# amiezzi/narrow_band_least_squares

Measured on AMD Instinct MI355X. Metric: (window x band) LTS solves/sec, 8-element synthetic, higher is better.
Workload: dtype f64

## Files before the change

include/nbls.h:

```cpp
#ifndef NBLS_H
#define NBLS_H

#include <stdint.h>

#ifdef __cplusplus
extern "C" {
#endif

typedef struct nbls_handle nbls_handle;

typedef enum {
    NBLS_OK = 0,
    NBLS_ERR_ARG = -1,
    NBLS_ERR_STATE = -2,
    NBLS_ERR_GEOMETRY = -3,
    NBLS_ERR_HIP = -4,
    NBLS_ERR_NOMEM = -5,
    NBLS_ERR_UNSUPPORTED = -6,
    NBLS_ERR_COMM = -7
} nbls_status;

typedef struct {
    double alpha;
    int32_t h;
// ... 82 lines not shown
int nbls_comm_unique_id(void* id, int32_t nbytes);
int nbls_comm_init_rank(nbls_handle* h, const void* id, int32_t world, int32_t rank);
int nbls_reserve_results(nbls_handle* h, int64_t bytes);
int nbls_comm_gather(nbls_handle* const* hs, int32_t n, int32_t root, int64_t block_bytes, int64_t status,
                     void* host_out, int64_t host_bytes);
int nbls_load_result_block(nbls_handle* h, const void* block, int64_t nbytes);
int nbls_comm_destroy(nbls_handle* h);

int nbls_set_option(nbls_handle* h, const char* key, int64_t value);
int nbls_developer_build(void);

enum {
    NBLS_ROUTE_REJECTED = 0,
    NBLS_ROUTE_SCREEN = 1,
    NBLS_ROUTE_MFMA = 2,
    NBLS_ROUTE_VALU_LDS = 3,
    NBLS_ROUTE_VALU_GLOBAL = 4
};
enum { NBLS_ROUTE_QUANTIZE = 0, NBLS_ROUTE_SCREEN_STAGE = 1, NBLS_ROUTE_VERIFY = 2, NBLS_ROUTE_GENERAL = 3 };
enum { NBLS_ROUTE_OPT_NC4 = 1, NBLS_ROUTE_OPT_NSL1 = 2, NBLS_ROUTE_OPT_TB8 = 4, NBLS_ROUTE_OPT_TB4 = 8 };
typedef struct {
    int32_t correlator;
    int32_t impl;
    int32_t ncopy, G, S, nsl;
    int32_t PFB, CSB, CSA, WP;
    int32_t screen_inst;
    int32_t tab_lds;
    int32_t quant_inst;
    int32_t quant_waves;
    int32_t verifier;
    int32_t verify_threads;
    int64_t lds_dyn[4];
    int64_t lds_static[4];
} nbls_route;
int nbls_route_xcorr(int32_t nelem, int32_t W, int32_t npairs, int32_t vrows, int64_t npts_pad, int32_t xcorr_impl,
                     int32_t flags, nbls_route* out);
int nbls_route_table(int32_t nelem, int32_t W0, int32_t W1, int32_t npairs, int32_t vrows, int64_t npts_pad,
                     int32_t xcorr_impl, int32_t flags, nbls_route* out);

int nbls_set_profiling(nbls_handle* h, int32_t on);
int nbls_get_timings(nbls_handle* h, nbls_timings* out);

int nbls_run(nbls_handle* h, int32_t nbands, const double* sos, int32_t nsections,
             int32_t zero_phase, const double* taper_left, const double* taper_right,
             int32_t taper_len, const int32_t* winlen, const int32_t* wininc,
             int32_t vector_len, const nbls_lts_params* lts, int32_t xcorr_impl,
             double* vel, double* baz, double* mdccm, double* sigma_tau, int32_t* nwin,
             int32_t* lag, double* cmax, uint8_t* weights, double* z);

int nbls_probe_mfma_f64(nbls_handle* h, const double* a, const double* b, double* out);
int nbls_probe_mfma_i8(nbls_handle* h, const int32_t* a, const int32_t* b, int32_t* out);

int nbls_debug_screen_stats(nbls_handle* h, int64_t* out8);
int nbls_debug_lts_stamps(nbls_handle* h, double* out8);
int nbls_debug_lts_coop_breakdown(nbls_handle* h, double* out8);
int nbls_debug_screen_stamps(nbls_handle* h, double* out10);

#ifdef __cplusplus
}
#endif
#endif
```

narrow_band_least_squares_amd/_hip.py:

```python
import ctypes as C
import os

import numpy as np

_HERE = os.path.dirname(os.path.abspath(__file__))
LIB_PATH = os.environ.get('NBLS_LIB') or os.path.join(_HERE, 'csrc', 'libnbls_hip.so')

EXPORTS = [
    'nbls_version', 'nbls_device_count', 'nbls_create', 'nbls_destroy', 'nbls_last_error', 'nbls_set_trace',
    'nbls_set_geometry', 'nbls_plan', 'nbls_execute', 'nbls_execute_stages', 'nbls_execute_after', 'nbls_set_trace_shape', 'nbls_upload_rows', 'nbls_sync',
    'nbls_fetch', 'nbls_fetch_filtered', 'nbls_device_results', 'nbls_set_profiling',
    'nbls_get_timings', 'nbls_run', 'nbls_probe_mfma_f64', 'nbls_probe_mfma_i8', 'nbls_debug_screen_stats', 'nbls_set_window_ranges', 'nbls_debug_screen_stamps', 'nbls_debug_lts_stamps',
    'nbls_set_trace_rows', 'nbls_result_layout', 'nbls_fetch_packed', 'nbls_comm_init_all', 'nbls_comm_unique_id',
    'nbls_comm_init_rank', 'nbls_reserve_results', 'nbls_comm_gather', 'nbls_comm_destroy', 'nbls_set_option',
    'nbls_developer_build', 'nbls_set_trace_from', 'nbls_debug_lts_coop_breakdown', 'nbls_filter_segment',
    'nbls_set_filtered', 'nbls_load_result_block', 'nbls_stream_results', 'nbls_result_batches', 'nbls_wait_result_batch',
    'nbls_comm_set_library', 'nbls_set_uncertainty', 'nbls_fetch_uncertainty', 'nbls_expect_upload', 'nbls_abort_upload',
    'nbls_set_segments', 'nbls_route_xcorr', 'nbls_route_table',
]

NBLS_ERR_ARG, NBLS_ERR_STATE, NBLS_ERR_GEOMETRY = -1, -2, -3
NBLS_ERR_HIP, NBLS_ERR_NOMEM, NBLS_ERR_UNSUPPORTED, NBLS_ERR_COMM = -4, -5, -6, -7


class NblsError(RuntimeError):
    def __init__(self, code, msg):
        super().__init__('libnbls_hip error %d: %s' % (code, msg))
        self.code = code


class LtsParams(C.Structure):
    _fields_ = [
        ('alpha', C.c_double), ('h', C.c_int32), ('nstarts', C.c_int32),
        ('starts', C.POINTER(C.c_int32)), ('csteps', C.c_int32), ('csteps2', C.c_int32),
        ('ncand', C.c_int32), ('xij_mad', C.c_double * 2), ('raw_factor', C.c_double),
        ('rew_table', C.POINTER(C.c_double)), ('quantile', C.c_double), ('zero_scale', C.c_double),
    ]


class Timings(C.Structure):
    _fields_ = [('filter_ms', C.c_double), ('xcorr_ms', C.c_double), ('solve_ms', C.c_double),
                ('total_ms', C.c_double), ('xcorr_launches', C.c_int64), ('quantize_ms', C.c_double),
                ('screen_ms', C.c_double), ('verify_ms', C.c_double), ('xcorr_impl', C.c_int32),
                ('xcorr_fallback_bands', C.c_int32)]


ROUTE_REJECTED, ROUTE_SCREEN, ROUTE_MFMA, ROUTE_VALU_LDS, ROUTE_VALU_GLOBAL = 0, 1, 2, 3, 4
ROUTE_QUANTIZE, ROUTE_SCREEN_STAGE, ROUTE_VERIFY, ROUTE_GENERAL = 0, 1, 2, 3
ROUTE_OPT_NC4, ROUTE_OPT_NSL1, ROUTE_OPT_TB8, ROUTE_OPT_TB4 = 1, 2, 4, 8
ROUTE_DTYPE = np.dtype([(k, np.int32) for k in ('correlator', 'impl', 'ncopy', 'G', 'S', 'nsl', 'PFB', 'CSB', 'CSA', 'WP',
                                                 'screen_inst', 'tab_lds', 'quant_inst', 'quant_waves', 'verifier',
                                                 'verify_threads')] +
                       [('lds_dyn', np.int64, (4,)), ('lds_static', np.int64, (4,))])
ROUTE_KEYS = ('correlator', 'ncopy', 'G', 'S', 'nsl', 'screen_inst', 'tab_lds', 'quant_inst', 'quant_waves', 'verifier',
              'verify_threads')


class Route(C.Structure):
    _fields_ = [(k, C.c_int32) for k in ROUTE_DTYPE.names[:16]] + [('lds_dyn', C.c_int64 * 4), ('lds_static', C.c_int64 * 4)]


_lib = None


def load_library(path=None):
    global _lib
    if _lib is not None and path is None:
        return _lib
    p = path or LIB_PATH
    if not os.path.exists(p):
        raise ImportError('%s not found: build it with `make -C %s` (or __graft_entry__.build()); '
# ... 2 lines not shown
    dp = C.POINTER(C.c_double)
    ip = C.POINTER(C.c_int32)
    u8p = C.POINTER(C.c_uint8)
    vp = C.c_void_p
    lib.nbls_version.restype = C.c_int
    lib.nbls_create.argtypes = [C.c_int, C.POINTER(vp)]
    lib.nbls_destroy.argtypes = [vp]
    lib.nbls_destroy.restype = None
    lib.nbls_last_error.argtypes = [vp]
    lib.nbls_last_error.restype = C.c_char_p
    lib.nbls_set_trace.argtypes = [vp, dp, C.c_int32, C.c_int64, C.c_double]
    lib.nbls_set_trace_rows.argtypes = [vp, C.POINTER(C.c_void_p), C.c_int32, C.c_int64, C.c_double]
    lib.nbls_result_layout.argtypes = [vp, C.POINTER(C.c_int64)]
    lib.nbls_fetch_packed.argtypes = [vp, C.c_void_p, C.c_int64]
    lib.nbls_comm_init_all.argtypes = [C.POINTER(vp), C.c_int32]
    lib.nbls_comm_unique_id.argtypes = [C.c_void_p, C.c_int32]
    lib.nbls_comm_init_rank.argtypes = [vp, C.c_void_p, C.c_int32, C.c_int32]
    lib.nbls_reserve_results.argtypes = [vp, C.c_int64]
    lib.nbls_load_result_block.argtypes = [vp, C.c_void_p, C.c_int64]
    lib.nbls_comm_gather.argtypes = [C.POINTER(vp), C.c_int32, C.c_int32, C.c_int64, C.c_int64, C.c_void_p, C.c_int64]
    lib.nbls_comm_destroy.argtypes = [vp]
    lib.nbls_expect_upload.argtypes = [vp]
    lib.nbls_abort_upload.argtypes = [vp]
    lib.nbls_comm_set_library.argtypes = [C.c_char_p, C.c_int32]
    lib.nbls_set_uncertainty.argtypes = [vp, dp]
    lib.nbls_fetch_uncertainty.argtypes = [vp, dp, dp]
    lib.nbls_stream_results.argtypes = [vp, C.c_int32]
    lib.nbls_result_batches.argtypes = [vp, C.POINTER(C.c_int32)]
    lib.nbls_wait_result_batch.argtypes = [vp, C.c_int32, C.POINTER(C.c_int64), C.POINTER(C.c_void_p)]
    lib.nbls_set_trace_from.argtypes = [vp, vp]
    lib.nbls_filter_segment.argtypes = [vp, C.c_int32, dp, dp]
    lib.nbls_set_filtered.argtypes = [vp, C.c_int32, dp]
    lib.nbls_set_option.argtypes = [vp, C.c_char_p, C.c_int64]
    lib.nbls_set_geometry.argtypes = [vp, dp, ip, dp, C.c_int32]
    plan_args = [vp, C.c_int32, dp, C.c_int32, C.c_int32, dp, dp, C.c_int32, ip, ip, C.c_int32,
                 C.POINTER(LtsParams), C.c_int32]
    lib.nbls_plan.argtypes = plan_args
    lib.nbls_execute.argtypes = [vp]
    lib.nbls_execute_stages.argtypes = [vp, C.c_int32]
    lib.nbls_execute_after.argtypes = [vp, vp]
    lib.nbls_set_trace_shape.argtypes = [vp, C.c_int32, C.c_int64, C.c_double]
    lib.nbls_upload_rows.argtypes = [vp, C.POINTER(C.c_void_p), C.c_int32, C.c_int64]
    lib.nbls_sync.argtypes = [vp]
    fetch_args = [dp, dp, dp, dp, ip, ip, dp, u8p, dp]
    lib.nbls_fetch.argtypes = [vp] + fetch_args
    lib.nbls_fetch_filtered.argtypes = [vp, C.c_int32, dp]
    lib.nbls_device_results.argtypes = [vp, C.POINTER(vp), C.POINTER(C.c_int64)]
    lib.nbls_set_profiling.argtypes = [vp, C.c_int32]
    lib.nbls_get_timings.argtypes = [vp, C.POINTER(Timings)]
    lib.nbls_run.argtypes = plan_args + fetch_args
    lib.nbls_probe_mfma_f64.argtypes = [vp, dp, dp, dp]
    lib.nbls_probe_mfma_i8.argtypes = [vp, ip, ip, ip]
    lib.nbls_debug_screen_stats.argtypes = [vp, C.POINTER(C.c_int64)]
    lib.nbls_set_window_ranges.argtypes = [vp, C.c_int32, ip, ip]
    lib.nbls_set_segments.argtypes = [vp, C.c_int32]
    lib.nbls_debug_screen_stamps.argtypes = [vp, dp]
    lib.nbls_debug_lts_stamps.argtypes = [vp, dp]
    lib.nbls_debug_lts_coop_breakdown.argtypes = [vp, dp]
    lib.nbls_route_xcorr.argtypes = [C.c_int32, C.c_int32, C.c_int32, C.c_int32, C.c_int64, C.c_int32, C.c_int32,
                                     C.POINTER(Route)]
    lib.nbls_route_table.argtypes = [C.c_int32, C.c_int32, C.c_int32, C.c_int32, C.c_int32, C.c_int64, C.c_int32, C.c_int32,
                                     C.c_void_p]
    for name in EXPORTS:
        if name not in ('nbls_destroy', 'nbls_last_error'):
            getattr(lib, name).restype = C.c_int
    if path is None:
        _lib = lib
    return lib


def _dptr(a):
    return None if a is None else a.ctypes.data_as(C.POINTER(C.c_double))


def _iptr(a):
    return None if a is None else a.ctypes.data_as(C.POINTER(C.c_int32))


def _u8ptr(a):
    return None if a is None else a.ctypes.data_as(C.POINTER(C.c_uint8))


def _f64(a):
    return np.ascontiguousarray(a, dtype=np.float64)


class Handle:

    def __init__(self, device_id=0):
        self.lib = load_library()
        h = C.c_void_p()
        rc = self.lib.nbls_create(int(device_id), C.byref(h))
        if rc != 0:
            raise NblsError(rc, self.lib.nbls_last_error(None).decode())
        self._h = h
        self.device_id = int(device_id)
        self.nchans = self.npts = self.npairs = 0
        self.nbands = self.vector_len = 0
        self.nseg = 1
        self._keep = []
        self.profiling = False
        self.resident_key = None

    def close(self):
        if getattr(self, '_h', None):
            self.lib.nbls_destroy(self._h)
# ... 314 lines not shown
```

narrow_band_least_squares_amd/csrc/api.hip:

```cpp
#include "nbls_internal.h"
#include <algorithm>

#include <cmath>
#include <cstdio>
#include <cstdlib>
#include <cstring>
#include <chrono>
#include <condition_variable>
#include <functional>
#include <mutex>
#include <thread>
#include <unistd.h>

namespace {

std::mutex g_err_mu;
std::string g_err;

int fail(nbls_handle* h, int code, const std::string& msg) {
    if (h) { std::lock_guard<std::mutex> l(h->err_mu); h->err = msg; }
    else { std::lock_guard<std::mutex> l(g_err_mu); g_err = msg; }
    return code;
}

// ... 294 lines not shown
    for (int i = 0; i < 4; ++i) if (h->ev[i]) (void)hipEventDestroy(h->ev[i]);
    for (hipEvent_t e : h->bev) (void)hipEventDestroy(e);
    for (hipEvent_t e : h->pev) (void)hipEventDestroy(e);
    for (hipEvent_t e : h->rev) (void)hipEventDestroy(e);
    if (h->cstream) { (void)hipStreamSynchronize(h->cstream); (void)hipStreamDestroy(h->cstream); }
    if (h->ustream) { (void)hipStreamSynchronize(h->ustream); (void)hipStreamDestroy(h->ustream); }
    for (hipEvent_t e : h->uev) (void)hipEventDestroy(e);
    if (h->ev_uprev) (void)hipEventDestroy(h->ev_uprev);
    if (h->h_res) (void)hipHostFree(h->h_res);
    if (h->ev_xd) (void)hipEventDestroy(h->ev_xd);
    if (h->ev_plan) (void)hipEventDestroy(h->ev_plan);
    if (h->ev_up) (void)hipEventDestroy(h->ev_up);
    if (h->up && h->up != h->stream) (void)hipStreamDestroy(h->up);
    if (h->stream2) (void)hipStreamDestroy(h->stream2);
    if (h->stream) (void)hipStreamDestroy(h->stream);
    if (h->stage) (void)hipHostFree(h->stage);
    delete h;
}

static void set_elements(nbls_handle* h, int32_t nchans) {
    const int E = h->nseg > 1 && nchans % h->nseg == 0 ? nchans / h->nseg : nchans;
    if (h->nelem != E && h->d_xij) {
        (void)hipFree(h->d_xij); h->d_xij = nullptr;
        h->caps.erase((const void*)&h->d_xij);
        h->npairs = 0;
    }
    h->nelem = E;
}

static int trace_shape_impl(nbls_handle* h, int32_t nchans, int64_t npts, double fs) {
    HIPCHK(h, hipSetDevice(h->device));
    const int64_t pad = (npts + 63) / 64 * 64;
    const size_t need = (size_t)nchans * pad * sizeof(double);
    if (!h->d_trace || h->cap_trace < need) {
        if (h->d_trace) { (void)hipFree(h->d_trace); h->d_trace = nullptr; h->cap_trace = 0; }
        HIPCHK(h, hipMalloc((void**)&h->d_trace, need));
        h->cap_trace = need;
    }
    set_elements(h, nchans);
    h->nchans = nchans;
    h->npts = npts;
    h->npts_pad = pad;
    h->fs = fs;
    h->planned = false;
    h->trace_loaded = false;
    h->rows_landed.store(0, std::memory_order_release);
    h->upload_state.store(2, std::memory_order_release);
    return NBLS_OK;
}

static int trace_copy_impl(nbls_handle* h, const double* const* rows, const double* flat) {
    struct Guard {
        nbls_handle* h; bool ok = false;
        ~Guard() { h->upload_state.store(ok ? 0 : -1, std::memory_order_release); }
    } guard{h};
    h->rows_landed.store(0, std::memory_order_release);
    h->upload_state.store(1, std::memory_order_release);
    HIPCHK(h, hipSetDevice(h->device));
    const int32_t nchans = h->nchans;
    const int64_t npts = h->npts, pad = h->npts_pad;
    if (!h->ustream) HIPCHK(h, hipStreamCreateWithFlags(&h->ustream, hipStreamNonBlocking));
    if (!h->ev_uprev) HIPCHK(h, hipEventCreateWithFlags(&h->ev_uprev, hipEventDisableTiming));
    while ((int)h->uev.size() < nchans) {
        hipEvent_t e;
        HIPCHK(h, hipEventCreateWithFlags(&e, hipEventDisableTiming));
        h->uev.push_back(e);
    }
    for (hipStream_t s : {h->stream, h->stream2}) {
        if (!s) continue;
        HIPCHK(h, hipEventRecord(h->ev_uprev, s));
        HIPCHK(h, hipStreamWaitEvent(h->ustream, h->ev_uprev, 0));
    }
    if (pad > npts)
        HIPCHK(h, hipMemset2DAsync(h->d_trace + npts, pad * sizeof(double), 0, (pad - npts) * sizeof(double), nchans, h->ustream));
    if (flat) {
        HIPCHK(h, hipMemcpy2DAsync(h->d_trace, pad * sizeof(double), flat, npts * sizeof(double),
                                   npts * sizeof(double), nchans, hipMemcpyHostToDevice, h->ustream));
        for (int c = 0; c < nchans; ++c) HIPCHK(h, hipEventRecord(h->uev[c], h->ustream));
        h->rows_landed.store(nchans, std::memory_order_release);
    } else {
        for (int c = 0; c < nchans; ++c) {
            HIPCHK(h, hipMemcpyAsync(h->d_trace + (size_t)c * pad, rows[c], npts * sizeof(double), hipMemcpyHostToDevice, h->ustream));
            HIPCHK(h, hipEventRecord(h->uev[c], h->ustream));
            h->rows_landed.store(c + 1, std::memory_order_release);
        }
    }
    HIPCHK(h, hipStreamSynchronize(h->ustream));
    h->trace_loaded = true;
    guard.ok = true;
    return NBLS_OK;
}

static int wait_rows(nbls_handle* h, int done) {
    const auto t0 = std::chrono::steady_clock::now();
    for (long spin = 0;; ++spin) {
        const int st = h->upload_state.load(std::memory_order_acquire);
        const int landed = h->rows_landed.load(std::memory_order_acquire);
        if (st < 0) return -1;
        if (st == 0) return h->trace_loaded ? h->nchans : -1;
        if (st == 2) return -3;
        if (landed > done) return landed;
        if ((spin & 1023) == 1023 && std::chrono::steady_clock::now() - t0 > std::chrono::seconds(120)) return -2;
        std::this_thread::yield();
    }
}

static int set_trace_impl(nbls_handle* h, const double* const* rows, const double* flat, int32_t nchans, int64_t npts,
                          double fs) {
    const int rc = trace_shape_impl(h, nchans, npts, fs);
    return rc ? rc : trace_copy_impl(h, rows, flat);
}

int nbls_set_trace_shape(nbls_handle* h, int32_t nchans, int64_t npts, double fs) {
    if (!h) return NBLS_ERR_ARG;
    if (nchans < 1 || npts < 1 || !(fs > 0.0)) return fail(h, NBLS_ERR_ARG, "nbls_set_trace_shape: bad argument");
    return trace_shape_impl(h, nchans, npts, fs);
}

int nbls_upload_rows(nbls_handle* h, const double* const* rows, int32_t nchans, int64_t npts) {
    if (!h) return NBLS_ERR_ARG;
    if (!rows || nchans != h->nchans || npts != h->npts || !h->d_trace)
        return fail(h, NBLS_ERR_ARG, "nbls_upload_rows: rows do not match the shape declared with nbls_set_trace_shape");
    for (int c = 0; c < nchans; ++c)
        if (!rows[c]) return fail(h, NBLS_ERR_ARG, "nbls_upload_rows: null row");
    return trace_copy_impl(h, rows, nullptr);
}

int nbls_expect_upload(nbls_handle* h) {
    if (!h) return NBLS_ERR_ARG;
    int declared = 2;
    if (!h->upload_state.compare_exchange_strong(declared, 3, std::memory_order_acq_rel))
        return fail(h, NBLS_ERR_STATE, "nbls_expect_upload: no trace shape declared (nbls_set_trace_shape) or its samples are there already");
    return NBLS_OK;
}

int nbls_abort_upload(nbls_handle* h) {
    if (!h) return NBLS_ERR_ARG;
    int st = h->upload_state.load(std::memory_order_acquire);
    while ((st == 2 || st == 3) && !h->upload_state.compare_exchange_weak(st, -1, std::memory_order_acq_rel)) {}
    return NBLS_OK;
}

int nbls_set_trace(nbls_handle* h, const double* trace, int32_t nchans, int64_t npts, double fs) {
    if (!h) return NBLS_ERR_ARG;
    if (!trace || nchans < 1 || npts < 1 || !(fs > 0.0)) return fail(h, NBLS_ERR_ARG, "nbls_set_trace: bad argument");
    return set_trace_impl(h, nullptr, trace, nchans, npts, fs);
}

int nbls_set_trace_from(nbls_handle* h, const nbls_handle* src) {
    if (!h || !src) return NBLS_ERR_ARG;
    if (!src->d_trace) return fail(h, NBLS_ERR_STATE, "nbls_set_trace_from: the source handle has no trace");
    if (h == src) return NBLS_OK;
    if (h->device != src->device) return fail(h, NBLS_ERR_ARG, "nbls_set_trace_from: handles are on different devices");
    HIPCHK(h, hipSetDevice(h->device));
    const size_t need = (size_t)src->nchans * src->npts_pad * sizeof(double);
    if (!h->d_trace || h->cap_trace < need) {
        if (h->d_trace) { (void)hipFree(h->d_trace); h->d_trace = nullptr; h->cap_trace = 0; }
        HIPCHK(h, hipMalloc((void**)&h->d_trace, need));
        h->cap_trace = need;
    }
    {
        nbls_handle* s_ = const_cast<nbls_handle*>(src);
        int landed = 0;
        while (landed >= 0 && landed < src->nchans) landed = wait_rows(s_, landed);
        if (landed < 0) return fail(h, NBLS_ERR_STATE, "nbls_set_trace_from: the source handle's trace did not arrive");
        if (!src->uev.empty() && (int)src->uev.size() >= src->nchans) HIPCHK(h, hipStreamWaitEvent(h->stream, src->uev[src->nchans - 1], 0));
    }
    HIPCHK(h, hipMemcpyAsync(h->d_trace, src->d_trace, need, hipMemcpyDeviceToDevice, h->stream));
    set_elements(h, src->nchans);
    h->nchans = src->nchans;
    h->npts = src->npts;
    h->npts_pad = src->npts_pad;
    h->fs = src->fs;
    h->planned = false;
    h->trace_loaded = true;
    h->rows_landed.store(h->nchans, std::memory_order_release);
    h->upload_state.store(0, std::memory_order_release);
    return NBLS_OK;
}

int nbls_set_trace_rows(nbls_handle* h, const double* const* rows, int32_t nchans, int64_t npts, double fs) {
    if (!h) return NBLS_ERR_ARG;
    if (!rows || nchans < 1 || npts < 1 || !(fs > 0.0)) return fail(h, NBLS_ERR_ARG, "nbls_set_trace_rows: bad argument");
    for (int c = 0; c < nchans; ++c)
        if (!rows[c]) return fail(h, NBLS_ERR_ARG, "nbls_set_trace_rows: NULL row pointer");
    return set_trace_impl(h, rows, nullptr, nchans, npts, fs);
}

int nbls_set_geometry(nbls_handle* h, const double* xij, const int32_t* pair_idx, const double* xpinv,
                      int32_t npairs) {
    if (!h) return NBLS_ERR_ARG;
    if (!xij || !pair_idx || !xpinv) return fail(h, NBLS_ERR_ARG, "nbls_set_geometry: NULL pointer");
// ... 293 lines not shown
            xs[2 * k] = h->h_xij[2 * k] / lts->xij_mad[0];
            xs[2 * k + 1] = h->h_xij[2 * k + 1] / lts->xij_mad[1];
            xc[k] = xs[2 * k] * xs[2 * k + 1];
        }
        if ((rc = alloc_copy(h, &h->d_xs, xs.data(), xs.size()))) return rc;
        if ((rc = alloc_copy(h, &h->d_xc, xc.data(), xc.size()))) return rc;
        const int NS = (P + 3) / 4;
        std::vector<double> xss((size_t)(NS + 16) * 2, 0.0);
        for (int i = 0; i < NS; ++i) { xss[2 * i] = xs[2 * (4 * i)]; xss[2 * i + 1] = xs[2 * (4 * i) + 1]; }
        if ((rc = alloc_copy(h, &h->d_xss, xss.data(), xss.size()))) return rc;
    }
    h->arena_mode = false;
    if (h->stage && h->d_parena && h->stage_used)
        HIPCHK(h, hipMemcpyAsync(h->d_parena, h->stage, h->stage_used, hipMemcpyHostToDevice, h->up));
    h->planned = true;
    if (h->opt.plan_timing) {
        const auto tp3 = std::chrono::steady_clock::now();
        auto ms = [](auto a, auto b) { return std::chrono::duration<double, std::milli>(b - a).count(); };
        fprintf(stderr, "nbls_plan: tables %.3f ms, uploads %.3f ms, buffers+rest %.3f ms\n", ms(tp0, tp1), ms(tp1, tp2), ms(tp2, tp3));
    }
    return NBLS_OK;
}

int nbls_execute(nbls_handle* h) { return nbls_execute_stages(h, 7); }

int nbls_execute_after(nbls_handle* h, nbls_handle* prev) {
    if (!h || !prev || prev == h) return NBLS_ERR_ARG;
    if (prev->device != h->device) return fail(h, NBLS_ERR_ARG, "nbls_execute_after: the two handles are on different devices");
    if (!prev->ev_xd || !prev->ev_xd_recorded) return fail(h, NBLS_ERR_STATE, "nbls_execute_after: the other handle has not queued a pass");
    h->after = prev;
    const int rc = nbls_execute_stages(h, 7);
    h->after = nullptr;
    return rc;
}

int nbls_execute_stages(nbls_handle* h, int32_t stage_mask) {
    if (!h) return NBLS_ERR_ARG;
    if (!h->planned) return fail(h, NBLS_ERR_STATE, "nbls_execute: no plan");
    if ((stage_mask & 6) && !h->d_xij) return fail(h, NBLS_ERR_STATE, "nbls_execute: no geometry set");
    const int upload_st = h->upload_state.load(std::memory_order_acquire);
    if (!((stage_mask & 1) && (upload_st == 1 || upload_st == 3)) && !h->trace_loaded)
        return fail(h, NBLS_ERR_STATE, "nbls_execute: the trace was declared (nbls_set_trace_shape) but not uploaded");
    HIPCHK(h, hipSetDevice(h->device));
    wait_uploads(h);
    h->work_queued = true;
    const size_t cells = (size_t)h->nbands * h->vector_len;
    const int P = h->d_xij ? h->npairs : 1;
    (void)cells; (void)P;
    if (!h->rbatches.empty() && h->cstream) HIPCHK(h, hipStreamWaitEvent(h->stream, h->rev[2 * (h->rbatches.size() - 1) + 1], 0));
    h->rbatches.clear();
    HIPCHK(h, hipMemsetAsync(h->d_res, 0, h->res_bytes, h->stream));
    if (h->prof) HIPCHK(h, hipEventRecord(h->ev[0], h->stream));
    if (stage_mask & 1) {
        for (int done = 0; done < h->nchans;) {
            int landed = wait_rows(h, done);
            if (landed < 0 || landed <= done)
                return fail(h, NBLS_ERR_STATE, landed == -2 ? "nbls_execute: the announced trace did not arrive (no nbls_upload_rows within 120 s)"
                                               : landed == -3 ? "nbls_execute: the trace was declared (nbls_set_trace_shape) but not uploaded"
                                                              : "nbls_execute: the upload of the trace failed");
            if (h->opt.filter_row_step > 0 && landed > done + h->opt.filter_row_step) landed = done + h->opt.filter_row_step;
            if ((int)h->uev.size() >= landed) HIPCHK(h, hipStreamWaitEvent(h->stream, h->uev[landed - 1], 0));
            HIPCHK(h, nbls_launch_filter(h, done, landed - done));
            done = landed;
        }
    }
    if (h->prof) HIPCHK(h, hipEventRecord(h->ev[1], h->stream));
    h->solve_done = false;
    h->last_stage_mask = stage_mask;
    h->fuse_solve = ((stage_mask & 6) == 6) && h->xcorr_impl == 3 && (h->opt.overlap > 0 || h->stream_results);
    int64_t nbatch_est = 0;
    for (const nbls_wgroup& g : h->wgroups)
        if (g.u1 > g.u0) nbatch_est += g.screen && h->screen_batch > 0 ? (g.u1 - g.u0 + h->screen_batch - 1) / h->screen_batch : 1;
    const bool small_batches = nbatch_est > 1 && h->nunits / nbatch_est < 1024;
    h->solve_on_stream2 = h->fuse_solve && h->stream2 && (h->opt.overlap > 0 || (h->opt.overlap == 0 && h->stream_results && small_batches));
    if (h->stream_results) {
        if (!h->cstream) HIPCHK(h, hipStreamCreateWithFlags(&h->cstream, hipStreamNonBlocking));
        if (h->cap_hres < h->res_bytes) {
            HIPCHK(h, hipStreamSynchronize(h->cstream));
            if (h->h_res) { (void)hipHostFree(h->h_res); h->h_res = nullptr; h->cap_hres = 0; }
            HIPCHK(h, hipHostMalloc((void**)&h->h_res, h->res_bytes ? h->res_bytes : 8, hipHostMallocDefault));
            h->cap_hres = h->res_bytes ? h->res_bytes : 8;
        }
    }
    if (h->after && (stage_mask & 2)) HIPCHK(h, hipStreamWaitEvent(h->stream, h->after->ev_xd, 0));
    h->ev_xd_by_launcher = false;
    if (stage_mask & 2) HIPCHK(h, nbls_launch_xcorr(h));
    if (h->ev_xd && (stage_mask & 2) && !h->ev_xd_by_launcher) { HIPCHK(h, hipEventRecord(h->ev_xd, h->stream)); h->ev_xd_recorded = true; }
    if (h->prof) HIPCHK(h, hipEventRecord(h->ev[2], h->stream));
    if ((stage_mask & 4) && !h->solve_done) HIPCHK(h, nbls_launch_solve(h));
    if (h->prof) { HIPCHK(h, hipEventRecord(h->ev[3], h->stream)); h->ev_valid = true; }
    if (h->stream_results && h->rbatches.empty()) HIPCHK(h, nbls_queue_result_batch(h, 0, h->nunits, h->stream));
    return NBLS_OK;
}

}

hipError_t nbls_queue_result_batch(nbls_handle* h, int64_t u0, int64_t u1, hipStream_t producer) {
    if (!h->stream_results || !h->cstream || !h->h_res) return hipSuccess;
    const size_t k = h->rbatches.size();
    while (h->rev.size() < 2 * (k + 1)) {
        hipEvent_t e;
        hipError_t ce = hipEventCreateWithFlags(&e, hipEventDisableTiming);
        if (ce != hipSuccess) return ce;
        h->rev.push_back(e);
    }
    nbls_handle::result_batch rb{u0, u1, 0, 0};
    if (u1 > u0) {
        auto cell = [&](int64_t u) {
            const int b = (int)(std::upper_bound(h->unit_off.begin(), h->unit_off.end(), (int32_t)u) - h->unit_off.begin()) - 1;
            const int64_t first = (int)h->woff.size() == h->nbands ? h->woff[b] : 0;
            return (int64_t)b * h->vector_len + first + (u - h->unit_off[b]);
        };
        rb.c0 = cell(u0);
        rb.c1 = cell(u1 - 1) + 1;
    }
    hipError_t e = hipEventRecord(h->rev[2 * k], producer);
    if (e != hipSuccess) return e;
    if ((e = hipStreamWaitEvent(h->cstream, h->rev[2 * k], 0)) != hipSuccess) return e;
    if (rb.c1 > rb.c0) {
        const size_t cells = (size_t)h->nbands * h->vector_len;
        for (int g = 0; g < 4; ++g) {
            const size_t off = ((size_t)g * cells + (size_t)rb.c0) * sizeof(double);
            if ((e = hipMemcpyAsync(h->h_res + off, h->d_res + off, (size_t)(rb.c1 - rb.c0) * sizeof(double), hipMemcpyDeviceToHost, h->cstream)) != hipSuccess) return e;
        }
        const size_t moff = 4 * cells * sizeof(double) + (size_t)rb.c0 * h->mask_bytes;
        if ((e = hipMemcpyAsync(h->h_res + moff, h->d_res + moff, (size_t)(rb.c1 - rb.c0) * h->mask_bytes, hipMemcpyDeviceToHost, h->cstream)) != hipSuccess) return e;
    }
// ... 298 lines not shown
    }
    return fail(h, NBLS_ERR_ARG, std::string("unknown option '") + key + "'");
}

int nbls_developer_build(void) {
#ifdef NBLS_DEVELOPER
    return 1;
#else
    return 0;
#endif
}

int nbls_set_profiling(nbls_handle* h, int32_t on) {
    if (!h) return NBLS_ERR_ARG;
    h->prof = on != 0;
    return NBLS_OK;
}

int nbls_get_timings(nbls_handle* h, nbls_timings* out) {
    if (!h || !out) return NBLS_ERR_ARG;
    *out = h->tim;
    return NBLS_OK;
}

int nbls_run(nbls_handle* h, int32_t nbands, const double* sos, int32_t nsections, int32_t zero_phase,
             const double* taper_left, const double* taper_right, int32_t taper_len, const int32_t* winlen,
             const int32_t* wininc, int32_t vector_len, const nbls_lts_params* lts, int32_t xcorr_impl,
             double* vel, double* baz, double* mdccm, double* sigma_tau, int32_t* nwin, int32_t* lag,
             double* cmax, uint8_t* weights, double* z) {
    int rc = nbls_plan(h, nbands, sos, nsections, zero_phase, taper_left, taper_right, taper_len, winlen,
                       wininc, vector_len, lts, xcorr_impl);
    if (rc) return rc;
    if ((rc = nbls_execute(h))) return rc;
    if ((rc = nbls_sync(h))) return rc;
    return nbls_fetch(h, vel, baz, mdccm, sigma_tau, nwin, lag, cmax, weights, z);
}

int nbls_probe_mfma_f64(nbls_handle* h, const double* a, const double* b, double* out) {
    if (!h || !a || !b || !out) return NBLS_ERR_ARG;
    HIPCHK(h, hipSetDevice(h->device));
    double *da = nullptr, *db = nullptr, *dout = nullptr;
    HIPCHK(h, hipMalloc((void**)&da, 64 * sizeof(double)));
    HIPCHK(h, hipMalloc((void**)&db, 64 * sizeof(double)));
    HIPCHK(h, hipMalloc((void**)&dout, 256 * sizeof(double)));
    HIPCHK(h, copy_sync(h, da, a, 64 * sizeof(double), hipMemcpyHostToDevice));
    HIPCHK(h, copy_sync(h, db, b, 64 * sizeof(double), hipMemcpyHostToDevice));
    HIPCHK(h, nbls_launch_probe_mfma(h, da, db, dout));
    HIPCHK(h, hipStreamSynchronize(h->stream));
    HIPCHK(h, copy_sync(h, out, dout, 256 * sizeof(double), hipMemcpyDeviceToHost));
    (void)hipFree(da); (void)hipFree(db); (void)hipFree(dout);
    return NBLS_OK;
}

int nbls_debug_screen_stats(nbls_handle* h, int64_t* out4) {
    if (!h || !out4) return NBLS_ERR_ARG;
    if (!h->d_cand || h->screen_batch <= 0) return fail(h, NBLS_ERR_STATE, "no screening run yet");
    HIPCHK(h, hipSetDevice(h->device));
    HIPCHK(h, hipStreamSynchronize(h->stream));
    const int N = h->nelem;
    const int64_t last = h->last_batch > 0 ? h->last_batch : h->nunits - ((h->nunits - 1) / h->screen_batch) * h->screen_batch;
    std::vector<int32_t> c((size_t)last * N * N * 32);
    HIPCHK(h, copy_sync(h, c.data(), h->d_cand, c.size() * sizeof(int32_t), hipMemcpyDeviceToHost));
    for (int q = 0; q < 8; ++q) out4[q] = 0;
    for (int64_t u = 0; u < last; ++u)
        for (int i = 0; i < N; ++i)
            for (int j = 0; j < N; ++j) {
                if (i == j) continue;
                const int32_t* e = &c[((u * N + i) * N + j) * 32];
                out4[0] += 1;
                out4[1] += e[1] != 0;
                out4[2] += e[0];
                if (e[0] > out4[3]) out4[3] = e[0];
                int n = e[0] < 26 ? e[0] : 26;
                int v[26];
                for (int q = 0; q < n; ++q) v[q] = e[6 + q];
                std::sort(v, v + n);
                for (int q = 0; q < n; ) {
                    int r = q + 1;
                    while (r < n && v[r] == v[r - 1] + 1) ++r;
                    out4[4] += 1;
                    if (r - q >= 2) out4[5] += r - q;
                    q = r;
                }
            }
    return NBLS_OK;
}

int nbls_debug_screen_stamps(nbls_handle* h, double* out6) {
    if (!h || !out6) return NBLS_ERR_ARG;
    if (!h->d_stamps) return fail(h, NBLS_ERR_STATE, "run with NBLS_SCREEN_STAMPS=1");
    HIPCHK(h, hipSetDevice(h->device));
    HIPCHK(h, hipStreamSynchronize(h->stream));
    const int64_t last = h->last_batch > 0 ? h->last_batch : h->nunits - ((h->nunits - 1) / h->screen_batch) * h->screen_batch;
    const int64_t nwg = ((last + 7) / 8) * 8 * h->nelem;
    std::vector<unsigned long long> st((size_t)nwg * 8);
    HIPCHK(h, copy_sync(h, st.data(), h->d_stamps, st.size() * sizeof(unsigned long long), hipMemcpyDeviceToHost));
    for (int i = 0; i < 10; ++i) out6[i] = 0.0;
    int64_t cnt = 0;
    for (int64_t g = 0; g < nwg; ++g) {
        const unsigned long long* s = &st[(size_t)g * 8];
        if (s[5] <= s[0] || s[5] - s[0] > 100000000ull) continue;
        for (int i = 0; i < 5; ++i) out6[i] += (double)(s[i + 1] - s[i]);
        out6[5] += (double)(s[5] - s[0]);
        out6[6] += (double)(s[6] & 0xffffffffull);
        out6[7] += (double)(s[6] >> 32);
        out6[8] += (double)(s[7] & 0xffffffffull);
// ... 60 lines not shown
```

narrow_band_least_squares_amd/csrc/filter.hip:

```cpp
#include "nbls_internal.h"
#include "wave_ops.h"
#include <cstdlib>
#include <type_traits>

namespace {

constexpr int C = NBLS_FILTER_CHUNK;
constexpr int T = NBLS_FILTER_TILE;
constexpr int G = NBLS_FILTER_GROUP;

struct FilterArgs {
    const double* in;
    int64_t in_stride;
    int in_mod;
    double* out;
    int64_t out_stride;
    const double* sos;
    const double* fw;
    const double* mpow;
    double* cstate;
    double* gend;
    double* gin;
    int nchans;
    int nseries;
// ... 429 lines not shown
    FilterArgs a;
    a.nchans = h->nchans;
    a.nseries = h->fbands * h->nchans;
    a.ch0 = 0;
    a.nch = h->nchans;
    a.nsub = a.nseries;
    a.npts = h->npts;
    a.nchunks = h->nchunks;
    a.ngroups = (int)((h->nchunks + G - 1) / G);
    a.sos = h->d_sos;
    a.fw = h->d_fw;
    a.mpow = h->d_M;
    a.cstate = h->d_cstate;
    a.gend = h->d_gend;
    a.gin = h->d_gin;
    a.tl = h->d_tl;
    a.tr = h->d_tr;
    a.taper_len = 0;
    a.final_pass = 0;
    a.cstate_next = nullptr;
    a.tstate = nullptr;
    a.recompute = 0;
    a.init = d_init;
    a.fin = d_fin;
    a.out = h->d_filt;
    a.out_stride = h->npts_pad;
    if (!reverse) {
        a.in = h->d_trace;
        a.in_stride = h->npts_pad;
        a.in_mod = h->nchans;
        a.reverse = 0;
        a.plen = h->npts;
    } else {
        a.in = h->d_filt;
        a.in_stride = h->npts_pad;
        a.in_mod = a.nseries;
        a.reverse = 1;
        a.plen = h->nchunks * C;
    }
    return run_pass<S>(h, a, false);
}

__global__ void copy_taper_kernel(const double* in, double* out, int64_t stride, int64_t npts, int nchans,
                                  const double* tl, const double* tr, int taper_len) {
    const int64_t g = (int64_t)blockIdx.x * blockDim.x + threadIdx.x;
    const int ch = blockIdx.y;
    if (g >= npts || ch >= nchans) return;
    double v = in[ch * stride + g];
    if (g < taper_len) v = v * tl[g];
    else if (g >= npts - taper_len) v = v * tr[g - (npts - taper_len)];
    out[ch * stride + g] = v;
}

}

hipError_t nbls_launch_filter_segment(nbls_handle* h, int reverse, const double* d_init, double* d_fin) {
    switch (h->nsections) {
        case 1: return run_filter_segment<1>(h, reverse, d_init, d_fin);
        case 2: return run_filter_segment<2>(h, reverse, d_init, d_fin);
        case 3: return run_filter_segment<3>(h, reverse, d_init, d_fin);
        case 4: return run_filter_segment<4>(h, reverse, d_init, d_fin);
        case 5: return run_filter_segment<5>(h, reverse, d_init, d_fin);
        case 6: return run_filter_segment<6>(h, reverse, d_init, d_fin);
        case 7: return run_filter_segment<7>(h, reverse, d_init, d_fin);
        case 8: return run_filter_segment<8>(h, reverse, d_init, d_fin);
        default: return hipErrorInvalidValue;
    }
}

hipError_t nbls_launch_filter(nbls_handle* h, int ch0, int nch) {
    if (ch0 < 0 || nch < 1 || ch0 + nch > h->nchans) return hipErrorInvalidValue;
    if (h->nsections == 0) {
        hipLaunchKernelGGL(copy_taper_kernel, dim3((unsigned)((h->npts + 255) / 256), nch), dim3(256), 0,
                           h->stream, h->d_trace + (size_t)ch0 * h->npts_pad, h->d_filt + (size_t)ch0 * h->npts_pad, h->npts_pad,
                           h->npts, nch, h->d_tl, h->d_tr, h->taper_len);
        return hipGetLastError();
    }
    switch (h->nsections) {
        case 1: return run_filter<1>(h, ch0, nch);
        case 2: return run_filter<2>(h, ch0, nch);
        case 3: return run_filter<3>(h, ch0, nch);
        case 4: return run_filter<4>(h, ch0, nch);
        case 5: return run_filter<5>(h, ch0, nch);
        case 6: return run_filter<6>(h, ch0, nch);
        case 7: return run_filter<7>(h, ch0, nch);
        case 8: return run_filter<8>(h, ch0, nch);
        default: return hipErrorInvalidValue;
    }
}
```

narrow_band_least_squares_amd/csrc/nbls_internal.h:

```cpp
#pragma once
#include <hip/hip_runtime.h>
#include <stdint.h>
#include <atomic>
#include <mutex>
#include <string>
#include <unordered_map>
#include <unordered_set>
#include <vector>
#include "../../include/nbls.h"

#define NBLS_MAX_SECTIONS 8
#define NBLS_FILTER_CHUNK 512
#define NBLS_FILTER_TILE 16
#define NBLS_FILTER_GROUP 64
#define NBLS_MAX_PAIRS 512
#define NBLS_MAX_STARTS 1024
#define NBLS_MAX_CAND 16
#define NBLS_SLDS_XCORR_SIMPLE 80
#define NBLS_SLDS_VERIFY 16640
#define NBLS_SCREEN_TB 4

struct nbls_options {
    int lts_impl = 0;
    int lts_generic_h = 0;
    int lts_coop_threads = 0;
    int lts_sample_its = 0;
    int screen_nsl1 = 0;
    int screen_tb4 = 0;
    int screen_static = 0;
    int screen_pretest = 0;
    int screen_cxx = 0;
    int screen_nc4 = 0;
    int screen_tb8 = 0;
    int screen_batch_mb = 192;
    int solve_min_units = 0;
    int filter_row_step = 0;
    int result_tail_units = 0;
    int overlap = 0;
    int filter_nofuse = 0;
    int filter_nomfma = 0;
    int ablate = 0;
    int screen_stamps = 0;
    int screen_seed = 0;
    int lts_stamps = 0;
    int screen_pad_kb = 0;
    int lts_pad_kb = 0;
    int plan_timing = 0;
};

struct nbls_wgroup { int b0, b1, W; int64_t u0, u1; bool screen; };

struct nbls_handle {
    int device = 0;
    nbls_options opt;
    hipStream_t stream = nullptr;
    hipStream_t stream2 = nullptr;
    hipEvent_t ev_xd = nullptr;
    bool ev_xd_recorded = false;
    hipEvent_t ev_plan = nullptr;
    bool ev_xd_by_launcher = false;
    nbls_handle* after = nullptr;
    int num_cus = 0;
    hipStream_t up = nullptr;
    int stream_priority = 0;
    std::vector<hipEvent_t> pev;
    bool fuse_solve = false;
    bool solve_on_stream2 = false;
    bool solve_done = false;
    int last_stage_mask = 7;

    bool stream_results = false;
    unsigned char* h_res = nullptr;
    size_t cap_hres = 0;
    hipStream_t cstream = nullptr;
    struct result_batch { int64_t u0, u1, c0, c1; };
    std::vector<result_batch> rbatches;
    std::vector<hipEvent_t> rev;
    std::string err;
    std::mutex err_mu;
    bool trace_loaded = false;
    hipStream_t ustream = nullptr;
    std::vector<hipEvent_t> uev;
    hipEvent_t ev_uprev = nullptr;
    std::atomic<int> rows_landed{0};
    std::atomic<int> upload_state{0};

    double* d_trace = nullptr;
    size_t cap_trace = 0;
    int nchans = 0;
    int nseg = 1;
    int nelem = 0;
    int64_t npts = 0, npts_pad = 0;
    double fs = 0.0;

    int npairs = 0;
    double* d_xij = nullptr;
    int32_t* d_pair = nullptr;
    double* d_xpinv = nullptr;
    std::vector<double> h_xij;
    std::vector<double> h_tl, h_tr;
    std::vector<int32_t> h_pair;
    std::vector<double> h_xpinv;

    bool planned = false;
    int fbands = 0;
    int nbands = 0, nsections = 0, zero_phase = 0, taper_len = 0, vector_len = 0, xcorr_impl = 0;
    std::vector<int32_t> W, inc, nwin, unit_off;
    int64_t nunits = 0;
    int maxW = 0;
    int uniW = 0;
    int64_t nchunks = 0;
    double* d_sos = nullptr;
    double* d_M = nullptr;
    double* d_fw = nullptr;
    double* d_gend = nullptr;
    double* d_gin = nullptr;
    size_t cap_gend = 0, cap_gin = 0;
    double* d_seg_state = nullptr;
    size_t cap_seg_state = 0;
    double* d_tl = nullptr;
    double* d_tr = nullptr;
    int32_t* d_W = nullptr;
    int32_t* d_inc = nullptr;
    int32_t* d_nwin = nullptr;
    int32_t* d_unit_off = nullptr;
    int32_t* d_win_off = nullptr;
    std::vector<int32_t> win_first, win_count;
    int32_t* d_unit_band = nullptr;
    int32_t* d_unit_win = nullptr;

    double* d_filt = nullptr;
    double* d_cstate = nullptr;
    double* d_cstate2 = nullptr;
    size_t cap_cstate2 = 0;
    double* d_tstate = nullptr;
    size_t cap_tstate = 0;
    int32_t* d_lag = nullptr;
    double* d_cmax = nullptr;
// ... 16 lines not shown
    double unc_par[6] = {0, 0, 0, 0, 0, 0};
    double* d_unc = nullptr;
    size_t cap_unc = 0;
    double* d_z = nullptr;
    uint8_t* d_wts = nullptr;
    size_t cap_filt = 0, cap_cstate = 0, cap_lag = 0, cap_cmax = 0, cap_z = 0, cap_wts = 0;
    std::unordered_map<const void*, size_t> caps;
    unsigned char* stage = nullptr;
    size_t stage_cap = 0, stage_used = 0;
    hipEvent_t ev_up = nullptr;
    bool up_pending = false, stage_bypass = false;
    std::vector<double> hp_M, hp_FW;
    std::vector<int32_t> hp_ub, hp_uw;
    std::vector<int32_t> woff;
    bool work_queued = false;
    unsigned char* d_parena = nullptr;
    bool arena_mode = false;
    std::unordered_set<const void*> arena_owned;

    int8_t* d_qbuf = nullptr;
    double* d_qmeta = nullptr;
    int32_t* d_cand = nullptr;
    size_t cap_qbuf = 0, cap_qmeta = 0, cap_cand = 0;
    int64_t screen_batch = 0;
    int screen_wp = 0;
    int64_t last_batch = 0;
    std::vector<nbls_wgroup> wgroups;
    int skew_n = -1, skew_s = -1;
    int skew_o[32] = {0};
    int64_t lts_stamp_waves = 0;
    unsigned long long* d_stamps = nullptr;
    size_t cap_stamps = 0;

    bool lts = false;
    nbls_lts_params ltsp{};
    int32_t* d_starts = nullptr;
    double* d_rew = nullptr;
    double* d_xs = nullptr;
    double* d_xss = nullptr;
    double* d_xc = nullptr;
    size_t cap_starts = 0;

    bool prof = false;
    hipEvent_t ev[4] = {nullptr, nullptr, nullptr, nullptr};
    bool ev_valid = false;
    std::vector<hipEvent_t> bev;
    int bev_used = 0;
    bool prof_fused = false;
    int xcorr_impl_used = 0;
    nbls_timings tim{};
};

hipError_t nbls_launch_filter(nbls_handle* h, int ch0, int nch);
hipError_t nbls_launch_filter_segment(nbls_handle* h, int reverse, const double* d_init, double* d_fin);
hipError_t nbls_launch_xcorr(nbls_handle* h);
hipError_t nbls_launch_solve(nbls_handle* h);
hipError_t nbls_launch_solve_range(nbls_handle* h, int64_t u0, int64_t nu, hipStream_t st);
hipError_t nbls_launch_pack_weights(nbls_handle* h, int64_t u0, int64_t nu, hipStream_t st);
hipError_t nbls_queue_result_batch(nbls_handle* h, int64_t u0, int64_t u1, hipStream_t producer);
hipError_t nbls_launch_probe_mfma(nbls_handle* h, const double* da, const double* db, double* dout);
struct nbls_route_query {
    int N, W, npairs, vrows;
    int64_t npts_pad;
    int impl, flags, pad_kb;
    bool no_screen;
};
void nbls_route_compute(const nbls_route_query& q, nbls_route* r);
nbls_route_query nbls_route_query_of(const nbls_handle* h, int W, int vrows, int impl, bool no_screen);
hipError_t nbls_launch_xcorr_screen_range(nbls_handle* h, int64_t ub, int64_t ue, int gW, int64_t* launches_io);
hipError_t nbls_xcorr_screen_finish(nbls_handle* h, int64_t launches);
hipError_t nbls_launch_probe_mfma_i8(nbls_handle* h, const int* da, const int* db, int* dout);
```

narrow_band_least_squares_amd/engine.py:

```python
import functools
import itertools
import operator
import os
import threading

import numpy as np

from . import planner
from ._hip import Handle
from .stream import start_datenum

try:
    from . import _nbls_host as _hostext
except ImportError:
    _hostext = None

_handles = {}

UPLOAD_OVERLAP = True
ROW_PIPELINE = True
ROW_PIPELINE_MIN_BYTES = 256 << 20
GROUP_ORDER = True
STREAM_PRIORITY = True
PIPELINE_SPLIT = None
KEY_THREADS = None


def default_device():
    for key in ('NBLS_DEVICE', 'LOCAL_RANK'):
        v = os.environ.get(key)
        if v is not None and v != '':
            return int(v)
    return 0


def get_handle(device=None, slot=0):
    dev = default_device() if device is None else int(device)
    key = (os.getpid(), dev, int(slot))
    h = _handles.get(key)
    if h is None:
        h = Handle(dev)
        if STREAM_PRIORITY:
            h.set_option('stream_priority', min(int(slot), 2) - 1)
        _handles[key] = h
    return h


def pipeline_groups(nwin, npairs=28):
    env = os.environ.get('NBLS_PIPELINE_GROUPS')
    nb = len(nwin)
    if env:
        return max(1, min(nb, int(env)))
    weight = max(1.0, float(npairs) / 28.0)
    return max(1, min(4, nb, int(np.sum(nwin) * weight) // 16000))


_graveyard = []


def release_later(*objs):
    _graveyard.append(objs)


def release_deferred():
    del _graveyard[:]


STREAM_MIN_UNITS = 16000


def streamed_default():
    if os.environ.get('NBLS_STREAM_RESULTS', '1') == '0':
        return False
    env = os.environ.get('NBLS_PIPELINE_GROUPS')
# ... 781 lines not shown
```

Before: 3.799 million.

## Size filter launch groups by occupancy and overlap solve with stream2

```diff
diff --git a/include/nbls.h b/include/nbls.h
--- a/include/nbls.h
+++ b/include/nbls.h
@@ -158,6 +158,9 @@
 int nbls_probe_mfma_i8(nbls_handle* h, const int32_t* a, const int32_t* b, int32_t* out);
 
 int nbls_debug_screen_stats(nbls_handle* h, int64_t* out8);
+int nbls_debug_filter_groups(int32_t nchans, int32_t fbands, int64_t nchunks, int32_t nsections, int32_t num_cus,
+                             int32_t apply_waves_per_simd, int32_t* sizes, int32_t* ngroups, int32_t* group_min);
+int nbls_debug_pass_info(nbls_handle* h, int64_t* out8);
 int nbls_debug_lts_stamps(nbls_handle* h, double* out8);
 int nbls_debug_lts_coop_breakdown(nbls_handle* h, double* out8);
 int nbls_debug_screen_stamps(nbls_handle* h, double* out10);
diff --git a/narrow_band_least_squares_amd/_hip.py b/narrow_band_least_squares_amd/_hip.py
--- a/narrow_band_least_squares_amd/_hip.py
+++ b/narrow_band_least_squares_amd/_hip.py
@@ -16,7 +16,7 @@
     'nbls_developer_build', 'nbls_set_trace_from', 'nbls_debug_lts_coop_breakdown', 'nbls_filter_segment',
     'nbls_set_filtered', 'nbls_load_result_block', 'nbls_stream_results', 'nbls_result_batches', 'nbls_wait_result_batch',
     'nbls_comm_set_library', 'nbls_set_uncertainty', 'nbls_fetch_uncertainty', 'nbls_expect_upload', 'nbls_abort_upload',
-    'nbls_set_segments', 'nbls_route_xcorr', 'nbls_route_table',
+    'nbls_set_segments', 'nbls_route_xcorr', 'nbls_route_table', 'nbls_debug_filter_groups', 'nbls_debug_pass_info',
 ]
 
 NBLS_ERR_ARG, NBLS_ERR_STATE, NBLS_ERR_GEOMETRY = -1, -2, -3
@@ -125,6 +125,8 @@
     lib.nbls_probe_mfma_f64.argtypes = [vp, dp, dp, dp]
     lib.nbls_probe_mfma_i8.argtypes = [vp, ip, ip, ip]
     lib.nbls_debug_screen_stats.argtypes = [vp, C.POINTER(C.c_int64)]
+    lib.nbls_debug_pass_info.argtypes = [vp, C.POINTER(C.c_int64)]
+    lib.nbls_debug_filter_groups.argtypes = [C.c_int32, C.c_int32, C.c_int64, C.c_int32, C.c_int32, C.c_int32, ip, ip, ip]
     lib.nbls_set_window_ranges.argtypes = [vp, C.c_int32, ip, ip]
     lib.nbls_set_segments.argtypes = [vp, C.c_int32]
     lib.nbls_debug_screen_stamps.argtypes = [vp, dp]
diff --git a/narrow_band_least_squares_amd/csrc/api.hip b/narrow_band_least_squares_amd/csrc/api.hip
--- a/narrow_band_least_squares_amd/csrc/api.hip
+++ b/narrow_band_least_squares_amd/csrc/api.hip
@@ -370,7 +370,7 @@
 static int trace_copy_impl(nbls_handle* h, const double* const* rows, const double* flat) {
     struct Guard {
         nbls_handle* h; bool ok = false;
-        ~Guard() { h->upload_state.store(ok ? 0 : -1, std::memory_order_release); }
+        ~Guard() { h->upload_state.store(ok ? 0 : -1, std::memory_order_release); h->up_cv.notify_all(); }
     } guard{h};
     h->rows_landed.store(0, std::memory_order_release);
     h->upload_state.store(1, std::memory_order_release);
@@ -396,11 +396,13 @@
                                    npts * sizeof(double), nchans, hipMemcpyHostToDevice, h->ustream));
         for (int c = 0; c < nchans; ++c) HIPCHK(h, hipEventRecord(h->uev[c], h->ustream));
         h->rows_landed.store(nchans, std::memory_order_release);
+        h->up_cv.notify_all();
     } else {
         for (int c = 0; c < nchans; ++c) {
             HIPCHK(h, hipMemcpyAsync(h->d_trace + (size_t)c * pad, rows[c], npts * sizeof(double), hipMemcpyHostToDevice, h->ustream));
             HIPCHK(h, hipEventRecord(h->uev[c], h->ustream));
             h->rows_landed.store(c + 1, std::memory_order_release);
+            h->up_cv.notify_all();
         }
     }
     HIPCHK(h, hipStreamSynchronize(h->ustream));
@@ -419,7 +421,9 @@
         if (st == 2) return -3;
         if (landed > done) return landed;
         if ((spin & 1023) == 1023 && std::chrono::steady_clock::now() - t0 > std::chrono::seconds(120)) return -2;
-        std::this_thread::yield();
+        if (spin < 64) { std::this_thread::yield(); continue; }
+        std::unique_lock<std::mutex> lk(h->up_mu);
+        h->up_cv.wait_for(lk, std::chrono::microseconds(50));
     }
 }
 
@@ -456,6 +460,7 @@
     if (!h) return NBLS_ERR_ARG;
     int st = h->upload_state.load(std::memory_order_acquire);
     while ((st == 2 || st == 3) && !h->upload_state.compare_exchange_weak(st, -1, std::memory_order_acq_rel)) {}
+    h->up_cv.notify_all();
     return NBLS_OK;
 }
 
@@ -855,16 +860,30 @@
     HIPCHK(h, hipMemsetAsync(h->d_res, 0, h->res_bytes, h->stream));
     if (h->prof) HIPCHK(h, hipEventRecord(h->ev[0], h->stream));
     if (stage_mask & 1) {
-        for (int done = 0; done < h->nchans;) {
-            int landed = wait_rows(h, done);
-            if (landed < 0 || landed <= done)
+        std::vector<int> groups;
+        h->filter_group_min = 0;
+        const bool racing = upload_st == 1 || upload_st == 3;
+        if (h->opt.filter_row_step > 0) {
+            for (int c = 0; c < h->nchans; c += h->opt.filter_row_step)
+                groups.push_back(h->nchans - c < h->opt.filter_row_step ? h->nchans - c : h->opt.filter_row_step);
+        } else if ((racing || h->opt.filter_row_step < 0) && h->nsections > 0) {
+            groups.resize((size_t)h->nchans);
+            groups.resize((size_t)nbls_filter_groups(h->nchans, h->fbands, h->nchunks, h->nsections, h->num_cus,
+                                                     nbls_filter_apply_occupancy(h), groups.data(), &h->filter_group_min));
+        } else
+            groups.push_back(h->nchans);
+        h->filter_launches = 0;
+        int done = 0;
+        for (const int g : groups) {
+            const int landed = wait_rows(h, done + g - 1);
+            if (landed < done + g)
                 return fail(h, NBLS_ERR_STATE, landed == -2 ? "nbls_execute: the announced trace did not arrive (no nbls_upload_rows within 120 s)"
                                                : landed == -3 ? "nbls_execute: the trace was declared (nbls_set_trace_shape) but not uploaded"
                                                               : "nbls_execute: the upload of the trace failed");
-            if (h->opt.filter_row_step > 0 && landed > done + h->opt.filter_row_step) landed = done + h->opt.filter_row_step;
-            if ((int)h->uev.size() >= landed) HIPCHK(h, hipStreamWaitEvent(h->stream, h->uev[landed - 1], 0));
-            HIPCHK(h, nbls_launch_filter(h, done, landed - done));
-            done = landed;
+            if ((int)h->uev.size() >= done + g) HIPCHK(h, hipStreamWaitEvent(h->stream, h->uev[done + g - 1], 0));
+            HIPCHK(h, nbls_launch_filter(h, done, g));
+            ++h->filter_launches;
+            done += g;
         }
     }
     if (h->prof) HIPCHK(h, hipEventRecord(h->ev[1], h->stream));
@@ -875,7 +894,7 @@
     for (const nbls_wgroup& g : h->wgroups)
         if (g.u1 > g.u0) nbatch_est += g.screen && h->screen_batch > 0 ? (g.u1 - g.u0 + h->screen_batch - 1) / h->screen_batch : 1;
     const bool small_batches = nbatch_est > 1 && h->nunits / nbatch_est < 1024;
-    h->solve_on_stream2 = h->fuse_solve && h->stream2 && (h->opt.overlap > 0 || (h->opt.overlap == 0 && h->stream_results && small_batches));
+    h->solve_on_stream2 = h->fuse_solve && h->stream2 && (h->opt.overlap > 0 || (h->opt.overlap == 0 && h->stream_results && (small_batches || !h->prof)));
     if (h->stream_results) {
         if (!h->cstream) HIPCHK(h, hipStreamCreateWithFlags(&h->cstream, hipStreamNonBlocking));
         if (h->cap_hres < h->res_bytes) {
@@ -1280,6 +1299,28 @@
     return NBLS_OK;
 }
 
+int nbls_debug_filter_groups(int32_t nchans, int32_t fbands, int64_t nchunks, int32_t nsections, int32_t num_cus,
+                             int32_t apply_waves_per_simd, int32_t* sizes, int32_t* ngroups, int32_t* group_min) {
+    if (nchans < 1 || fbands < 1 || nchunks < 1 || nsections < 0 || num_cus < 1 || !sizes || !ngroups) return NBLS_ERR_ARG;
+    int gmin = 0;
+    *ngroups = nbls_filter_groups(nchans, fbands, nchunks, nsections, num_cus, apply_waves_per_simd, sizes, &gmin);
+    if (group_min) *group_min = gmin;
+    return NBLS_OK;
+}
+
+int nbls_debug_pass_info(nbls_handle* h, int64_t* out8) {
+    if (!h || !out8) return NBLS_ERR_ARG;
+    out8[0] = h->solve_on_stream2 ? 1 : 0;
+    out8[1] = h->fuse_solve ? 1 : 0;
+    out8[2] = h->filter_launches;
+    out8[3] = h->filter_group_min;
+    out8[4] = h->apply_occ_key >= 0 ? h->apply_occ : -1;
+    out8[5] = h->num_cus;
+    out8[6] = h->prof ? 1 : 0;
+    out8[7] = h->nchunks;
+    return NBLS_OK;
+}
+
 int nbls_debug_screen_stats(nbls_handle* h, int64_t* out4) {
     if (!h || !out4) return NBLS_ERR_ARG;
     if (!h->d_cand || h->screen_batch <= 0) return fail(h, NBLS_ERR_STATE, "no screening run yet");
diff --git a/narrow_band_least_squares_amd/csrc/filter.hip b/narrow_band_least_squares_amd/csrc/filter.hip
--- a/narrow_band_least_squares_amd/csrc/filter.hip
+++ b/narrow_band_least_squares_amd/csrc/filter.hip
@@ -505,6 +505,70 @@
     out[ch * stride + g] = v;
 }
 
+template <int S>
+int apply_occupancy(nbls_handle* h) {
+    const bool fuse = h->zero_phase && !h->opt.filter_nofuse;
+    const bool recompute = fuse && h->d_tstate;
+    int occ = 0;
+    auto ask = [&](const void* fn) {
+        int nb = 0;
+        if (hipOccupancyMaxActiveBlocksPerMultiprocessor(&nb, fn, 64, 0) != hipSuccess || nb < 1) { (void)hipGetLastError(); return; }
+        const int per_simd = (nb + 3) / 4;
+        if (occ == 0 || per_simd < occ) occ = per_simd;
+    };
+    ask(recompute ? (const void*)filter_apply_kernel<S, 1> : (const void*)filter_apply_kernel<S, 0>);
+    if (h->zero_phase) ask(recompute ? (const void*)filter_apply_kernel<S, 2> : (const void*)filter_apply_kernel<S, 0>);
+    return occ;
+}
+
+}
+
+int nbls_filter_apply_occupancy(nbls_handle* h) {
+    const bool fuse = h->zero_phase && !h->opt.filter_nofuse;
+    const int key = h->nsections * 4 + (h->zero_phase ? 2 : 0) + ((fuse && h->d_tstate) ? 1 : 0);
+    if (h->apply_occ_key == key) return h->apply_occ;
+    int occ = 0;
+    switch (h->nsections) {
+        case 1: occ = apply_occupancy<1>(h); break;
+        case 2: occ = apply_occupancy<2>(h); break;
+        case 3: occ = apply_occupancy<3>(h); break;
+        case 4: occ = apply_occupancy<4>(h); break;
+        case 5: occ = apply_occupancy<5>(h); break;
+        case 6: occ = apply_occupancy<6>(h); break;
+        case 7: occ = apply_occupancy<7>(h); break;
+        case 8: occ = apply_occupancy<8>(h); break;
+        default: break;
+    }
+    h->apply_occ = occ;
+    h->apply_occ_key = key;
+    return occ;
+}
+
+int nbls_filter_groups(int nchans, int fbands, int64_t nchunks, int nsections, int num_cus, int apply_waves_per_simd, int* sizes,
+                       int* group_min) {
+    if (nchans < 1) return 0;
+    if (fbands < 1) fbands = 1;
+    if (nchunks < 1) nchunks = 1;
+    if (num_cus < 1) num_cus = 1;
+    if (apply_waves_per_simd < 1) apply_waves_per_simd = 8;
+    const int64_t slots = (int64_t)num_cus * 4 * apply_waves_per_simd;
+    const int64_t apply_waves = (nchunks + 63) / 64 * fbands;
+    int64_t gmin = (slots + apply_waves - 1) / apply_waves;
+    const int D = 2 * nsections;
+    if (nsections >= 1 && (16 % D) == 0) {
+        const int64_t rows = ((int64_t)fbands * D + 15) / 16;
+        const int64_t tiles = (nchunks + 15) / 16;
+        const int64_t want = (int64_t)4 * 2 * num_cus;
+        const int64_t gs = (want + rows * tiles - 1) / (rows * tiles);
+        if (gs > gmin) gmin = gs;
+    }
+    if (gmin < 1) gmin = 1;
+    if (group_min) *group_min = (int)(gmin > nchans ? nchans : gmin);
+    const int ng = gmin >= nchans ? 1 : (int)(nchans / gmin);
+    const int base = nchans / ng, rem = nchans % ng;
+    if (sizes)
+        for (int g = 0; g < ng; ++g) sizes[g] = base + (g >= ng - rem ? 1 : 0);
+    return ng;
 }
 
 hipError_t nbls_launch_filter_segment(nbls_handle* h, int reverse, const double* d_init, double* d_fin) {
diff --git a/narrow_band_least_squares_amd/csrc/nbls_internal.h b/narrow_band_least_squares_amd/csrc/nbls_internal.h
--- a/narrow_band_least_squares_amd/csrc/nbls_internal.h
+++ b/narrow_band_least_squares_amd/csrc/nbls_internal.h
@@ -2,6 +2,7 @@
 #include <hip/hip_runtime.h>
 #include <stdint.h>
 #include <atomic>
+#include <condition_variable>
 #include <mutex>
 #include <string>
 #include <unordered_map>
@@ -84,6 +85,11 @@
     hipEvent_t ev_uprev = nullptr;
     std::atomic<int> rows_landed{0};
     std::atomic<int> upload_state{0};
+    std::mutex up_mu;
+    std::condition_variable up_cv;
+    int apply_occ = 0, apply_occ_key = -1;
+    int filter_launches = 0;
+    int filter_group_min = 0;
 
     double* d_trace = nullptr;
     size_t cap_trace = 0;
@@ -206,6 +212,8 @@
 };
 
 hipError_t nbls_launch_filter(nbls_handle* h, int ch0, int nch);
+int nbls_filter_groups(int nchans, int fbands, int64_t nchunks, int nsections, int num_cus, int apply_waves_per_simd, int* sizes, int* group_min);
+int nbls_filter_apply_occupancy(nbls_handle* h);
 hipError_t nbls_launch_filter_segment(nbls_handle* h, int reverse, const double* d_init, double* d_fin);
 hipError_t nbls_launch_xcorr(nbls_handle* h);
 hipError_t nbls_launch_solve(nbls_handle* h);
diff --git a/narrow_band_least_squares_amd/engine.py b/narrow_band_least_squares_amd/engine.py
--- a/narrow_band_least_squares_amd/engine.py
+++ b/narrow_band_least_squares_amd/engine.py
@@ -19,7 +19,7 @@
 
 UPLOAD_OVERLAP = True
 ROW_PIPELINE = True
-ROW_PIPELINE_MIN_BYTES = 256 << 20
+ROW_PIPELINE_MIN_BYTES = 64 << 20
 GROUP_ORDER = True
 STREAM_PRIORITY = True
 PIPELINE_SPLIT = None
```

Measured after the change: 3.724 million. 0.98x the previous value.
